# evanwporter/SparseCholesky

Hardware: AMD Instinct MI355X
Metric: numeric-factorization fp64 GFLOP/s (F=sum colcount^2) (higher is better)
Workload: dtype f64

## Files before the change

sparsecholesky_amd/csrc/kernels.hip:

```cpp
#include <hip/hip_runtime.h>

#include <cstdint>
#include <type_traits>

#include "kernels.hpp"

namespace sc {

typedef double double4_t __attribute__((ext_vector_type(4)));

__device__ __forceinline__ void report_fail(int32_t* info, const int32_t* post, int32_t col_internal) {
    atomicMin(info, (post ? post[col_internal] : col_internal) + 1);
}

__device__ __forceinline__ int bnd_at(const int32_t* b, int k, int mbc) {
    const int klo = b[0], khi = b[1];
    return k <= klo ? b[2] : (k >= khi ? mbc : b[2 + k - klo]);
}

__device__ __forceinline__ int lower_bound_i32(const int32_t* a, int n, int v) {
    int lo = 0, hi = n;
    while (lo < hi) {
        int mid = (lo + hi) >> 1;
        if (a[mid] < v)
// ... 11 lines not shown
    const int tid = threadIdx.x;
    const int lane = tid & 63, wid = tid >> 6;
    const int c0 = P.sn_start[s];
    const int w = P.sn_start[s + 1] - c0;
    const int m = P.sn_m[s];
    const int mb = m - w;
    const int j0 = t.y * ASM_COLS;
    const int j1 = min(m, j0 + ASM_COLS);
    double* panel = P.panel_pool + P.panel_off[s];
    double* cbs = P.cb_pool + P.cb_off[s];
    for (int j = j0 + wid; j < j1; j += 4) {
        double* col = (j < w) ? panel + (int64_t)j * m : cbs + (int64_t)(j - w) * mb - w;
#pragma unroll 4
        for (int r = j + lane; r < m; r += 64) col[r] = 0.0;
    }
    __syncthreads();
    for (int j = j0 + wid; j < min(j1, w); j += 4) {
        const int64_t a0 = P.a_ptr[c0 + j], a1 = P.a_ptr[c0 + j + 1];
        for (int64_t q = a0 + lane; q < a1; q += 64) panel[(int64_t)j * m + P.a_pos[q]] = Ax[P.a_src[q]];
    }
    __syncthreads();
    for (int ci = P.child_ptr[s]; ci < P.child_ptr[s + 1]; ++ci) {
        const int c = P.child_list[ci];
        const int mbc = P.sn_m[c] - (P.sn_start[c + 1] - P.sn_start[c]);
        const int32_t* __restrict__ rel = P.relind + P.rel_ptr[c];
        const double* __restrict__ cb = P.cb_pool + P.cb_off[c];
        const int32_t* __restrict__ cbnd = P.col_bnd + P.cbk_ptr[c];
        const int jlo = bnd_at(cbnd, t.y, mbc), jhi = bnd_at(cbnd, t.y + 1, mbc);
        for (int jc = jlo + wid; jc < jhi; jc += 4) {
            const int pj = rel[jc];
            const double* __restrict__ src = cb + (int64_t)jc * mbc;
            double* dst = (pj < w) ? panel + (int64_t)pj * m : cbs + (int64_t)(pj - w) * mb - w;
#pragma unroll 4
            for (int ic = jc + lane; ic < mbc; ic += 64) dst[rel[ic]] += src[ic];
        }
        __syncthreads();
    }
}

constexpr int ASM_CCH = 32;
__global__ __launch_bounds__(256) void assemble_tile_kernel(DevPlan P, const int2* __restrict__ tasks,
                                                             const double* __restrict__ Ax,
                                                             const int2* __restrict__ lim) {
    __shared__ double T[ASM_COLS * ASM_ROWS];
    __shared__ const double* s_src[ASM_CCH];
    __shared__ const int32_t* s_rel[ASM_CCH];
    __shared__ int s_mbc[ASM_CCH], s_ilo[ASM_CCH], s_ihi[ASM_CCH], s_jlo[ASM_CCH];
    __shared__ int8_t s_pj[ASM_CCH][ASM_COLS];
    const int2 t = tasks[blockIdx.x];
    const int s = t.x;
    const int k = t.y >> 16;
    const int jb = t.y & 0xffff;
    const int tid = threadIdx.x;
    const int lane = tid & 63, wid = tid >> 6;
    const int c0 = P.sn_start[s];
    const int w = P.sn_start[s + 1] - c0;
    const int m = P.sn_m[s];
    const int mb = m - w;
    const int j0 = jb * ASM_COLS;
    const int j1 = min(m, j0 + ASM_COLS);
    const int r0 = k * ASM_ROWS, r1 = min(m, r0 + ASM_ROWS);
    const int2 cl = lim ? lim[blockIdx.x] : make_int2(0, m);
    double* panel = P.panel_pool + P.panel_off[s];
    double* cbs = P.cb_pool + P.cb_off[s];
    const int cp0 = P.child_ptr[s], cp1 = P.child_ptr[s + 1];
#pragma unroll
    for (int q = 0; q < ASM_COLS / 4; ++q)
#pragma unroll
        for (int r = lane; r < ASM_ROWS; r += 64) T[(wid + 4 * q) * ASM_ROWS + r] = 0.0;
    for (int j = j0 + wid; j < min(j1, w); j += 4) {
        const int64_t a0 = P.a_ptr[c0 + j], a1 = P.a_ptr[c0 + j + 1];
        for (int64_t q = a0 + lane; q < a1; q += 64) {
            const int p = P.a_pos[q];
            if (p >= r0 && p < r1) T[(j - j0) * ASM_ROWS + (p - r0)] = Ax[P.a_src[q]];
        }
    }
    for (int cb = cp0; cb < cp1; cb += ASM_CCH) {
        const int nc = min(ASM_CCH, cp1 - cb);
        if (cb > cp0) __syncthreads();
        if (tid < nc) {
            const int c = P.child_list[cb + tid];
            const int mbc = P.sn_m[c] - (P.sn_start[c + 1] - P.sn_start[c]);
            const int32_t* rel = P.relind + P.rel_ptr[c];
            const int32_t* bnd = P.rel_bnd + P.rb_ptr[c];
            const int32_t* cbnd = P.col_bnd + P.cbk_ptr[c];
            const int ilo = bnd_at(bnd, k, mbc), ihi = bnd_at(bnd, k + 1, mbc);
            const int jlo = bnd_at(cbnd, jb, mbc), jhi = bnd_at(cbnd, jb + 1, mbc);
            int pj[ASM_COLS];
#pragma unroll
            for (int l = 0; l < ASM_COLS; ++l) {
                const int pc = (jlo + l < jhi && ilo < ihi) ? rel[jlo + l] : -1;
                pj[l] = (pc >= cl.x && pc < cl.y) ? pc - j0 : -1;
            }
#pragma unroll
            for (int l = 0; l < ASM_COLS; ++l) s_pj[tid][l] = (int8_t)pj[l];
            s_src[tid] = P.cb_pool + P.cb_off[c];
            s_rel[tid] = rel;
            s_mbc[tid] = mbc;
            s_ilo[tid] = ilo;
            s_ihi[tid] = ihi;
            s_jlo[tid] = jlo;
        }
        __syncthreads();
        for (int i = 0; i < nc; ++i) {
            const int pjl = lane < ASM_COLS ? (int)s_pj[i][lane] : -1;
            uint64_t mask = __ballot(pjl >= 0 && (pjl & 3) == wid);
            if (!mask) continue;
            const int mbc = s_mbc[i], ilo = s_ilo[i], ihi = s_ihi[i], jlo = s_jlo[i];
            const double* __restrict__ src = s_src[i];
            const int32_t* __restrict__ rel = s_rel[i];
            int jc[4], tc[4];
#pragma unroll
            for (int q = 0; q < 4; ++q) {
                const int b = mask ? __builtin_ctzll(mask) : -1;
                jc[q] = b < 0 ? -1 : jlo + b;
                tc[q] = b < 0 ? 0 : __shfl(pjl, b);
                mask &= mask - 1;
            }
            double v[4][ASM_ROWS / 64];
            int rr[4][ASM_ROWS / 64];
#pragma unroll
            for (int q = 0; q < 4; ++q) {
                const int lo = max(jc[q], ilo) + lane;
#pragma unroll
                for (int ch = 0; ch < ASM_ROWS / 64; ++ch) {
                    const int ic = lo + 64 * ch;
                    const bool ok = jc[q] >= 0 && ic < ihi;
                    rr[q][ch] = ok ? rel[ic] : -1;
                    v[q][ch] = ok ? src[(int64_t)jc[q] * mbc + ic] : 0.0;
                }
            }
#pragma unroll
            for (int q = 0; q < 4; ++q)
#pragma unroll
                for (int ch = 0; ch < ASM_ROWS / 64; ++ch)
                    if (rr[q][ch] >= 0) T[tc[q] * ASM_ROWS + rr[q][ch] - r0] += v[q][ch];
        }
    }
    for (int j = j0 + wid; j < j1; j += 4) {
        if (j < cl.x || j >= cl.y) continue;
        double* col = (j < w) ? panel + (int64_t)j * m : cbs + (int64_t)(j - w) * mb - w;
        const double* Tc = T + (j - j0) * ASM_ROWS - r0;
        for (int r = max(r0, j) + lane; r < r1; r += 64) col[r] = Tc[r];
    }
}

__device__ __forceinline__ __amdgpu_buffer_rsrc_t buf_rsrc(const double* base, uint32_t nbytes = 0xffffffffu) {
    return __builtin_amdgcn_make_buffer_rsrc(const_cast<double*>(base), 0, (int)nbytes, 0x00020000);
}
constexpr int BUF_DEAD = 0x7ffffff0;
__device__ __forceinline__ double buf_ld(__amdgpu_buffer_rsrc_t rs, int voff, int soff) {
    return __builtin_bit_cast(double, __builtin_amdgcn_raw_buffer_load_b64(rs, voff, soff, 0));
}
__device__ __forceinline__ void buf_st(double v, __amdgpu_buffer_rsrc_t rs, int voff, int soff) {
    __builtin_amdgcn_raw_buffer_store_b64(__builtin_bit_cast(decltype(__builtin_amdgcn_raw_buffer_load_b64(rs, 0, 0, 0)), v), rs, voff, soff, 0);
}

__device__ __forceinline__ double readlane_f64(double v, int src) {
    const long long b = __double_as_longlong(v);
    const int lo = __builtin_amdgcn_readlane((int)(b & 0xffffffff), src);
    const int hi = __builtin_amdgcn_readlane((int)(b >> 32), src);
    return __longlong_as_double(((long long)hi << 32) | (unsigned int)lo);
}

template <int J>
__device__ __forceinline__ void trsm_steps(double (&r)[PNB], const double* Lc, const double* invd, int nb) {
    constexpr int LD = PNB + 2;
    if constexpr (J < PNB) {
        if (J < nb) {
            const double rj = r[J] * invd[J];
            r[J] = rj;
#pragma unroll
            for (int q = J + 1; q < PNB; ++q) r[q] = fma(-rj, Lc[J * LD + q], r[q]);
            trsm_steps<J + 1>(r, Lc, invd, nb);
        }
    }
}

__device__ __forceinline__ double rsqrt_f64(double d) {
    double y = __builtin_amdgcn_rsq(d);
    const double h = 0.5 * d;
    y = y * fma(-h * y, y, 1.5);
    y = y * fma(-h * y, y, 1.5);
    return y;
}

__device__ __forceinline__ int pk_col(int m, int j) { return j * m - ((j * (j - 1)) >> 1); }

__device__ __forceinline__ void lds_barrier() { asm volatile("s_waitcnt lgkmcnt(0)\n\ts_barrier" ::: "memory"); }

__device__ __forceinline__ void tile_map(int q, int T, int WT, int& bi, int& bj) {
    const int np = WT * T - WT * (WT - 1) / 2;
    if (q < np) {
        int c = 0, rem = q;
        while (rem >= T - c) {
            rem -= T - c;
            ++c;
        }
        bi = c + rem;
        bj = c;
        return;
    }
    const int r = q - np;
    int b = (int)((sqrtf(8.0f * (float)r + 1.0f) - 1.0f) * 0.5f);
    while (b * (b + 1) / 2 > r) --b;
    while ((b + 1) * (b + 2) / 2 <= r) ++b;
    bi = WT + b;
    bj = WT + r - b * (b + 1) / 2;
}

constexpr int COLB = 132;

template <int KT>
struct SmallRegs {
    double v[KT][16];
    int bi[KT], bj[KT];
};

template <int KT, int NT = 256>
__device__ __forceinline__ void small_tiles(SmallRegs<KT>& R, int m, int w) {
    const int T = (m + 3) >> 2, WT = (w + 3) >> 2, ntile = T * (T + 1) / 2;
#pragma unroll
    for (int k = 0; k < KT; ++k) {
        const int q = threadIdx.x + NT * k;
        int bi = -1, bj = -1;
        if (q < ntile) tile_map(q, T, WT, bi, bj);
        R.bi[k] = bi;
        R.bj[k] = bj;
    }
}

template <int KT>
__device__ __forceinline__ void small_load(SmallRegs<KT>& R, const double* F, int m) {
#pragma unroll
    for (int k = 0; k < KT; ++k)
#pragma unroll
        for (int r = 0; r < 4; ++r)
#pragma unroll
            for (int c = 0; c < 4; ++c) {
                const int i = 4 * R.bi[k] + r, j = 4 * R.bj[k] + c;
                R.v[k][r * 4 + c] = (R.bi[k] >= 0 && i < m && i >= j) ? F[pk_col(m, j) + i - j] : 0.0;
            }
}

template <int KT>
__device__ __forceinline__ void small_steps(SmallRegs<KT>& R, double* colbuf, int w, int32_t* info, const int32_t* post, int c0) {
    for (int J = 0, b = 0; J < w; J += 4, ++b) {
        double* cb = colbuf + (b & 1) * 4 * COLB;
        const int nb = min(4, w - J);
#pragma unroll
        for (int k = 0; k < KT; ++k)
            if (R.bj[k] == b) {
#pragma unroll
                for (int r = 0; r < 4; ++r) {
                    double* row = cb + 4 * (4 * R.bi[k] + r);
                    *reinterpret_cast<double2*>(row) = make_double2(R.v[k][r * 4], R.v[k][r * 4 + 1]);
                    *reinterpret_cast<double2*>(row + 2) = make_double2(R.v[k][r * 4 + 2], R.v[k][r * 4 + 3]);
                }
            }
        lds_barrier();
        double D[4][4];
#pragma unroll
        for (int r = 0; r < 4; ++r) {
            const double2 x01 = *reinterpret_cast<const double2*>(cb + 4 * (J + r));
            const double2 x23 = *reinterpret_cast<const double2*>(cb + 4 * (J + r) + 2);
            D[r][0] = x01.x;
            D[r][1] = x01.y;
            D[r][2] = x23.x;
            D[r][3] = x23.y;
        }
        double Ld[4][4], rc[4];
#pragma unroll
        for (int c = 0; c < 4; ++c) {
            double dd = D[c][c];
#pragma unroll
            for (int t = 0; t < c; ++t) dd = fma(-Ld[c][t], Ld[c][t], dd);
            if (c < nb && threadIdx.x == 0 && !(dd > 0.0)) report_fail(info, post, c0 + J + c);
            rc[c] = c < nb ? rsqrt_f64(dd) : 0.0;
            Ld[c][c] = dd * rc[c];
#pragma unroll
            for (int r = c + 1; r < 4; ++r) {
                double x = D[r][c];
#pragma unroll
                for (int t = 0; t < c; ++t) x = fma(-Ld[r][t], Ld[c][t], x);
                Ld[r][c] = x * rc[c];
            }
        }
        auto solve_row = [&](int row, double (&l)[4]) {
            const double2 x01 = *reinterpret_cast<const double2*>(cb + 4 * row);
            const double2 x23 = *reinterpret_cast<const double2*>(cb + 4 * row + 2);
            const double cr[4] = {x01.x, x01.y, x23.x, x23.y};
#pragma unroll
            for (int k = 0; k < 4; ++k) {
                double x = cr[k];
#pragma unroll
                for (int t = 0; t < k; ++t) x = fma(-l[t], Ld[k][t], x);
                l[k] = x * rc[k];
            }
        };
#pragma unroll
        for (int k = 0; k < KT; ++k) {
            const int bi = R.bi[k], bj = R.bj[k];
            if (bi < 0 || bj < b) continue;
            double lj[4][4];
#pragma unroll
            for (int c = 0; c < 4; ++c) solve_row(4 * bj + c, lj[c]);
// ... 764 lines not shown
                for (int c = 0; c < 4; ++c) {
                    const int i = 4 * R.bi[0] + r, j = 4 * R.bj[0] + c;
                    if (i >= j) Sd[PNB * j - j * (j - 1) / 2 + (i - j)] = (i == j) ? 1.0 / R.v[0][r * 4 + c] : R.v[0][r * 4 + c];
                }
        }
        const int row = r0 + tid;
        const __amdgpu_buffer_rsrc_t rs = buf_rsrc(pan + (int64_t)k0 * m, (uint32_t)m * PNB * 8u);
        const int voff = row < r1 ? row * 8 : BUF_DEAD;
        double r[PNB];
#pragma unroll
        for (int c = 0; c < PNB; ++c) r[c] = buf_ld(rs, voff, c * m * 8);
        __syncthreads();
        trsm64_full(r, S);
#pragma unroll
        for (int c = 0; c < PNB; ++c) buf_st(r[c], rs, voff, c * m * 8);
        return;
    }
    if (SC_POTRF_FAST)
        small_steps1_fast(R, colbuf, PNB, P.info, P.post, c0 + k0);
    else
        small_steps<1>(R, colbuf, PNB, P.info, P.post, c0 + k0);
    if (R.bi[0] >= 0) {
#pragma unroll
        for (int r = 0; r < 4; ++r)
#pragma unroll
            for (int c = 0; c < 4; ++c) {
                const int i = 4 * R.bi[0] + r, j = 4 * R.bj[0] + c;
                if (i >= j) Sd[PNB * j - j * (j - 1) / 2 + (i - j)] = (i == j) ? 1.0 / R.v[0][r * 4 + c] : R.v[0][r * 4 + c];
            }
    }
    const int row = r0 + tid;
    const __amdgpu_buffer_rsrc_t rs = buf_rsrc(pan + (int64_t)k0 * m, (uint32_t)m * PNB * 8u);
    const int voff = row < r1 ? row * 8 : BUF_DEAD;
    double r[PNB];
#pragma unroll
    for (int c = 0; c < PNB; ++c) r[c] = buf_ld(rs, voff, c * m * 8);
    __syncthreads();
    if (tid == 0) {
        const int k1 = k0 + PNB;
        const int nwg = (max(r1, k1 + 1) - k1 + TRSM_ROWS - 1) / TRSM_ROWS;
        const int old = __hip_atomic_fetch_add(arrive + (t.ctr - 1), 1, __ATOMIC_RELAXED, __HIP_MEMORY_SCOPE_AGENT);
        s_last = old == nwg - 1;
        if (old == nwg - 1) __hip_atomic_store(arrive + (t.ctr - 1), 0, __ATOMIC_RELAXED, __HIP_MEMORY_SCOPE_AGENT);
    }
    __syncthreads();
    if (s_last && R.bi[0] >= 0) {
#pragma unroll
        for (int rr = 0; rr < 4; ++rr)
#pragma unroll
            for (int c = 0; c < 4; ++c) {
                const int i = 4 * R.bi[0] + rr, j = 4 * R.bj[0] + c;
                if (i >= j) blk[(int64_t)j * m + i] = R.v[0][rr * 4 + c];
            }
    }
    trsm64_full(r, S);
#pragma unroll
    for (int c = 0; c < PNB; ++c) buf_st(r[c], rs, voff, c * m * 8);
}

#ifndef SC_PROBE_NOGATHER
#define SC_PROBE_NOGATHER 0
#endif
#ifndef SC_PROBE_NOK
#define SC_PROBE_NOK 0
#endif
template <int BT, int WM, int WN, int BK = 16, int GR = 64>
__device__ __forceinline__ void syrk_gather_epilogue(const GemmTask& T, const int64_t* __restrict__ gblk,
                                                     const GSeg* __restrict__ gseg, int row0, int col0,
                                                     double4_t (&acc)[BT / WM / 16][BT / WN / 16], double* smem) {
    constexpr int NW = WM * WN, NT = 64 * NW;
    constexpr int RTM = BT / WM / 16, RTN = BT / WN / 16;
    constexpr int GLD = GR + 1;
    constexpr int GQ = BT == 64 ? (GR == 32 ? 8 : 64 / NW) : SC_GATHER_Q;
    constexpr int SB = BT == 64 ? 4 : 1;
    constexpr int OPS = 2 * 2 * BK * (BT + 16);
    static_assert(BT * GLD <= OPS, "gather chunk fits the operand LDS");
    const int tid = threadIdx.x, lane = tid & 63, wid = tid >> 6;
    const int wr = wid / WN, wc = wid % WN;
    const int w = T.gw;
    const int mb = T.M;
    const int nb = (mb + 63) >> 6;
    const int64_t* __restrict__ blk = gblk + T.gb;
    const GSeg* __restrict__ seg = gseg;
    double* G = smem;
    double* __restrict__ C = T.C;
    const int64_t ldc = T.ldc;
    const __amdgpu_buffer_rsrc_t rc = buf_rsrc(C + (int64_t)col0 * ldc, (uint32_t)(min(BT, T.N - col0) * ldc * 8));
#pragma unroll 1
    for (int h = 0; h < BT / GR; ++h) {
        const int r0 = row0 + h * GR;
        const int rb = r0 >> 6;
        if (h) __syncthreads();
        for (int e = tid; e < BT * GLD; e += NT) G[e] = 0.0;
        __syncthreads();
        const int cb1 = min(min(nb, rb + 1), (col0 + BT) >> 6);
        for (int cbk = col0 >> 6; !SC_PROBE_NOGATHER && r0 < mb && cbk < cb1; ++cbk) {
            const int64_t bi = (int64_t)rb * (rb + 1) / 2 + cbk;
            const int64_t p0 = blk[bi], p1 = blk[bi + 1];
            for (int64_t pb = p0; pb < p1; pb += SB) {
                int prw[SB], pcl[SB];
#pragma unroll
                for (int q = 0; q < SB; ++q) {
                    prw[q] = -1;
                    pcl[q] = -1;
                    if (pb + q < p1) {
                        const GSeg& g = seg[pb + q];
                        const int ic = g.ilo + lane, jl = g.jlo + lane;
                        if (ic < g.ihi) prw[q] = g.rel[ic] - w - r0;
                        if (jl < g.jhi) pcl[q] = g.rel[jl] - w - col0;
                    }
                }
#pragma unroll
                for (int q = 0; q < SB; ++q) {
                    if (pb + q >= p1) break;
                    const GSeg& g = seg[pb + q];
                    const int ic = g.ilo + lane;
                    const int prow = prw[q] < GR ? prw[q] : -1;
                    const int mbc = g.mbc;
                    const double* __restrict__ cb = g.cb;
                    uint64_t mask = __ballot(pcl[q] >= 0 && pcl[q] % NW == wid);
                    while (mask) {
                        int jc[GQ], pc[GQ];
#pragma unroll
                        for (int u = 0; u < GQ; ++u) {
                            const int b = mask ? __builtin_ctzll(mask) : -1;
                            jc[u] = b < 0 ? -1 : g.jlo + b;
                            pc[u] = b < 0 ? 0 : __builtin_amdgcn_readlane(pcl[q], b);
                            mask &= mask - 1;
                        }
                        double v[GQ];
                        bool ok[GQ];
#pragma unroll
                        for (int u = 0; u < GQ; ++u) {
                            ok[u] = jc[u] >= 0 && prow >= 0 && ic >= jc[u];
                            const __amdgpu_buffer_rsrc_t rs = buf_rsrc(cb + (int64_t)max(jc[u], 0) * mbc, (uint32_t)mbc * 8u);
                            v[u] = buf_ld(rs, ok[u] ? ic * 8 : BUF_DEAD, 0);
                        }
#pragma unroll
                        for (int u = 0; u < GQ; ++u)
                            if (ok[u]) G[pc[u] * GLD + prow] += v[u];
                    }
                }
            }
        }
        __syncthreads();
        static_assert(GR % (BT / WM) == 0, "a wave's rows lie in one chunk");
        if ((wr * (BT / WM)) / GR == h) {
#pragma unroll
            for (int a = 0; a < RTM; ++a)
#pragma unroll
                for (int b = 0; b < RTN; ++b)
#pragma unroll
                    for (int r = 0; r < 4; ++r) {
                        const int lr = wr * (BT / WM) + a * 16 + MFMA_F64_ROW(lane, r);
                        const int lc = wc * (BT / WN) + b * 16 + (lane & 15);
                        G[lc * GLD + (lr - h * GR)] -= acc[a][b][r];
                    }
        }
        __syncthreads();
#pragma unroll 4
        for (int e = tid; e < BT * GR; e += NT) {
            const int lr = e % GR, lc = e / GR;
            const int gi = r0 + lr, gj = col0 + lc;
            const bool live = gi < T.M && gi >= gj && gj < T.N;
            buf_st(G[lc * GLD + lr], rc, live ? (int)((gi + (int64_t)(gj - col0) * ldc) * 8) : BUF_DEAD, 0);
        }
    }
}

template <int BT, int WM, int WN, int BK = 16, int GR = 64>
__device__ __forceinline__ void syrk_rmw_epilogue(const GemmTask& T, int row0, int col0,
                                                  double4_t (&acc)[BT / WM / 16][BT / WN / 16], double* smem) {
    constexpr int NW = WM * WN, NT = 64 * NW;
    constexpr int RTM = BT / WM / 16, RTN = BT / WN / 16;
    constexpr int GLD = GR + 1;
    constexpr int OPS = 2 * 2 * BK * (BT + 16);
    static_assert(BT * GLD <= OPS, "chunk fits the operand LDS");
    static_assert(GR % (BT / WM) == 0, "a wave's rows lie in one chunk");
    const int tid = threadIdx.x, lane = tid & 63, wid = tid >> 6;
    const int wr = wid / WN, wc = wid % WN;
    double* G = smem;
    const int64_t ldc = T.ldc;
    const __amdgpu_buffer_rsrc_t rc = buf_rsrc(T.C + (int64_t)col0 * ldc, (uint32_t)(min(BT, T.N - col0) * ldc * 8));
#pragma unroll 1
    for (int h = 0; h < BT / GR; ++h) {
        const int r0 = row0 + h * GR;
        if (h) __syncthreads();
#pragma unroll 4
        for (int e = tid; e < BT * GR; e += NT) {
            const int lr = e % GR, lc = e / GR;
            const int gi = r0 + lr, gj = col0 + lc;
            const bool live = gi < T.M && gi >= gj && gj < T.N;
            G[lc * GLD + lr] = buf_ld(rc, live ? (int)((gi + (int64_t)(gj - col0) * ldc) * 8) : BUF_DEAD, 0);
        }
        __syncthreads();
        if ((wr * (BT / WM)) / GR == h) {
#pragma unroll
            for (int a = 0; a < RTM; ++a)
#pragma unroll
                for (int b = 0; b < RTN; ++b)
#pragma unroll
                    for (int r = 0; r < 4; ++r) {
                        const int lr = wr * (BT / WM) + a * 16 + MFMA_F64_ROW(lane, r);
                        const int lc = wc * (BT / WN) + b * 16 + (lane & 15);
                        G[lc * GLD + (lr - h * GR)] -= acc[a][b][r];
                    }
        }
        __syncthreads();
#pragma unroll 4
        for (int e = tid; e < BT * GR; e += NT) {
            const int lr = e % GR, lc = e / GR;
            const int gi = r0 + lr, gj = col0 + lc;
            const bool live = gi < T.M && gi >= gj && gj < T.N;
            buf_st(G[lc * GLD + lr], rc, live ? (int)((gi + (int64_t)(gj - col0) * ldc) * 8) : BUF_DEAD, 0);
        }
    }
}

template <int BT, int WM, int WN, int BK = 16>
__device__ __forceinline__ void mfma_kloop(const double* __restrict__ A, int64_t lda, int K, int M, int N, int row0,
                                           int col0, double4_t (&acc)[BT / WM / 16][BT / WN / 16], double* smem) {
    static_assert(BK == 16 || BK == 8, "four-deep k sub-steps of the MFMA");
    constexpr int NT = 64 * WM * WN;
    constexpr int LDT = BT + 16;
    constexpr int RTM = BT / WM / 16, RTN = BT / WN / 16;
    double(*As)[BK * LDT] = reinterpret_cast<double(*)[BK * LDT]>(smem);
    double(*Bs)[BK * LDT] = reinterpret_cast<double(*)[BK * LDT]>(smem + 2 * BK * LDT);
    const int tid = threadIdx.x;
    const int lane = tid & 63;
    const int wid = tid >> 6;
    const int wr = wid / WN, wc = wid % WN;
    constexpr int PER = BT * BK / NT;
    double ra[PER], rb[PER];
    auto gload = [&](int k0) {
        const __amdgpu_buffer_rsrc_t rs = buf_rsrc(A + (int64_t)k0 * lda, (uint32_t)(min(BK, K - k0) * lda * 8));
#pragma unroll
        for (int q = 0; q < PER; ++q) {
            const int e = tid + q * NT;
            const int r = e % BT, kk = e / BT;
            const int gr = row0 + r, gc = col0 + r;
            ra[q] = buf_ld(rs, gr < M ? (int)((gr + kk * lda) * 8) : BUF_DEAD, 0);
            rb[q] = buf_ld(rs, gc < N ? (int)((gc + kk * lda) * 8) : BUF_DEAD, 0);
        }
    };
    auto sstore = [&](int buf) {
#pragma unroll
        for (int q = 0; q < PER; ++q) {
            const int e = tid + q * NT;
            const int r = e % BT, kk = e / BT;
            As[buf][kk * LDT + r] = ra[q];
            Bs[buf][kk * LDT + r] = rb[q];
        }
    };

    const int nk = (K + BK - 1) / BK;
    auto stage = [&](int kt, auto last) {
        constexpr bool LAST = decltype(last)::value;
        const int cur = kt & 1;
        if (!LAST) gload((kt + 1) * BK);
        double av[2][RTM], bv[2][RTN];
        auto lread = [&](int kk, int slot) {
            const int krow = kk + (lane >> 4);
#pragma unroll
            for (int a = 0; a < RTM; ++a)
                av[slot][a] = As[cur][krow * LDT + wr * (BT / WM) + a * 16 + (lane & 15)];
#pragma unroll
            for (int b = 0; b < RTN; ++b)
                bv[slot][b] = Bs[cur][krow * LDT + wc * (BT / WN) + b * 16 + (lane & 15)];
        };
        lread(0, 0);
#pragma unroll
        for (int kk = 0; kk < BK; kk += 4) {
            const int slot = (kk / 4) & 1;
            if (kk + 4 < BK) lread(kk + 4, slot ^ 1);
#pragma unroll
            for (int a = 0; a < RTM; ++a)
#pragma unroll
                for (int b = 0; b < RTN; ++b)
                    acc[a][b] = __builtin_amdgcn_mfma_f64_16x16x4f64(av[slot][a], bv[slot][b], acc[a][b], 0, 0, 0);
            if (!LAST && kk == BK - 8) sstore(cur ^ 1);
        }
        __syncthreads();
    };
    gload(0);
    sstore(0);
    __syncthreads();
    for (int kt = 0; kt + 1 < nk; ++kt) stage(kt, std::false_type {});
    if (nk > 0) stage(nk - 1, std::true_type {});
}

template <int BK>
__device__ __forceinline__ void panel_prefactor(const GemmTask& T, int32_t* info, const int32_t* post,
                                                double* smem) {
    static_assert(2 * 2 * BK * (64 + 16) >= 64 * 65 / 2, "the packed diagonal block fits the operand LDS");
    double4_t acc[2][2];
#pragma unroll
    for (int a = 0; a < 2; ++a)
#pragma unroll
        for (int b = 0; b < 2; ++b) acc[a][b] = (double4_t){0.0, 0.0, 0.0, 0.0};
    mfma_kloop<64, 2, 2, BK>(T.A, T.lda, T.K, T.M, T.N, 0, 0, acc, smem);
    const int tid = threadIdx.x, lane = tid & 63, wid = tid >> 6;
    const int wr = wid >> 1, wc = wid & 1;
    const int64_t ldc = T.ldc;
    double* __restrict__ F = smem;
    const __amdgpu_buffer_rsrc_t rc = buf_rsrc(T.C, (uint32_t)(64 * ldc * 8));
    double cv[2][2][4];
#pragma unroll
    for (int a = 0; a < 2; ++a)
#pragma unroll
        for (int b = 0; b < 2; ++b)
#pragma unroll
            for (int r = 0; r < 4; ++r) {
                const int gi = wr * 32 + a * 16 + MFMA_F64_ROW(lane, r), gj = wc * 32 + b * 16 + (lane & 15);
                cv[a][b][r] = buf_ld(rc, gi >= gj ? (int)((gi + (int64_t)gj * ldc) * 8) : BUF_DEAD, 0);
            }
#pragma unroll
    for (int a = 0; a < 2; ++a)
#pragma unroll
        for (int b = 0; b < 2; ++b)
#pragma unroll
            for (int r = 0; r < 4; ++r) {
                const int gi = wr * 32 + a * 16 + MFMA_F64_ROW(lane, r), gj = wc * 32 + b * 16 + (lane & 15);
                if (gi >= gj) F[pk_col(64, gj) + gi - gj] = cv[a][b][r] - acc[a][b][r];
            }
    __syncthreads();
    SmallRegs<1> R;
    small_tiles<1>(R, PNB, PNB);
    small_load<1>(R, F, PNB);
    __syncthreads();
    small_steps1_fast(R, smem, PNB, info, post, T.pf);
    if (R.bi[0] < 0) return;
#pragma unroll
    for (int r = 0; r < 4; ++r)
#pragma unroll
        for (int c = 0; c < 4; ++c) {
            const int i = 4 * R.bi[0] + r, j = 4 * R.bj[0] + c;
            if (i >= j) T.C[(int64_t)j * ldc + i] = R.v[0][r * 4 + c];
        }
}

template <int BT, int WM, int WN, int TAG, int EPI, int LEAN = 0, int PF = 0>
__device__ __forceinline__ void syrk_tile_body(const GemmTask* __restrict__ tasks, const int2* __restrict__ tiles,
                                               int bidx, const int64_t* __restrict__ gblk,
                                               const GSeg* __restrict__ gseg, int32_t* info = nullptr,
                                               const int32_t* post = nullptr) {
    constexpr int BK = LEAN ? 8 : 16;
    constexpr int LDT = BT + 16;
    constexpr int RTM = BT / WM / 16, RTN = BT / WN / 16;
    __shared__ __attribute__((aligned(16))) double smem[2 * 2 * BK * LDT];

    const int2 tl = tiles[bidx];
    const GemmTask T = tasks[tl.x];
    if constexpr (PF) {
        static_assert(BT == 64 && WM == 2 && WN == 2 && TAG == 0, "pre-factor on 64 x 64 panel-update tiles");
        if (tl.y < 0) {
            panel_prefactor<BK>(T, info, post, smem);
            return;
        }
    }
    const int ti = tl.y >> 16, tj = tl.y & 0xffff;
    const int row0 = ti * BT, col0 = tj * BT;

    const int wid = threadIdx.x >> 6;
    if (wid >= WM * WN / 2) __builtin_amdgcn_s_setprio(1);

    double4_t acc[RTM][RTN];
#pragma unroll
    for (int a = 0; a < RTM; ++a)
#pragma unroll
        for (int b = 0; b < RTN; ++b) acc[a][b] = (double4_t){0.0, 0.0, 0.0, 0.0};
    if (!(SC_PROBE_NOK && TAG == 1 && T.gs >= 0)) mfma_kloop<BT, WM, WN, BK>(T.A, T.lda, T.K, T.M, T.N, row0, col0, acc, smem);

    if constexpr (TAG == 1) {
        if (T.gs >= 0) {
            syrk_gather_epilogue<BT, WM, WN, BK, LEAN ? 32 : 64>(T, gblk, gseg, row0, col0, acc, smem);
            return;
        }
    }
    syrk_rmw_epilogue<BT, WM, WN, BK, LEAN ? 32 : 64>(T, row0, col0, acc, smem);
}

template <int BT, int WM, int WN, int TAG, int EPI, int LEAN = 0, int PF = 0>
__global__ __launch_bounds__(64 * WM * WN, LEAN ? (TAG ? 5 : 6) : 1) void syrk_mfma_kernel(const GemmTask* __restrict__ tasks,
                                                                  const int2* __restrict__ tiles,
                                                                  const int64_t* __restrict__ gblk,
                                                                  const GSeg* __restrict__ gseg, int32_t* info,
                                                                  const int32_t* post) {
    syrk_tile_body<BT, WM, WN, TAG, EPI, LEAN, PF>(tasks, tiles, blockIdx.x, gblk, gseg, info, post);
}

static int small_kt(int maxm) {
    const int T = (maxm + 3) / 4;
    return (T * (T + 1) / 2 + 255) / 256;
}

hipError_t launch_front_small(const DevPlan& P, const int32_t* nodes, int count, int maxm, bool seq,
                              const double* Ax, hipStream_t st) {
    if (count <= 0) return hipSuccess;
    const size_t lds = (size_t)maxm * (maxm + 1) / 2 * sizeof(double);
    const int kt = small_kt(maxm);
    const dim3 grid(seq ? 1 : count);
    const int sq = seq ? count : 0;
    if (kt <= 1)
        hipLaunchKernelGGL(front_small_kernel<1>, grid, dim3(256), lds, st, P, nodes, Ax, sq);
    else if (kt == 2)
        hipLaunchKernelGGL(front_small_kernel<2>, grid, dim3(256), lds, st, P, nodes, Ax, sq);
    else
        hipLaunchKernelGGL(front_small_kernel<3>, grid, dim3(256), lds, st, P, nodes, Ax, sq);
    return hipGetLastError();
}

hipError_t launch_front_chain(const DevPlan& P, const ChainPlan& C, int first, int count, int maxm,
                              const double* Ax, hipStream_t st) {
    if (count <= 0) return hipSuccess;
    if (count > CHAIN_MAXF || maxm > 128) return hipErrorInvalidValue;
    const int fsz = maxm * (maxm + 1) / 2;
    const size_t lds = (size_t)fsz * sizeof(double);
    hipLaunchKernelGGL(chain_init_kernel, dim3(count), dim3(256), lds, st, P, C, first, Ax);
    hipLaunchKernelGGL(front_chain_kernel, dim3(1), dim3(CHAIN_NT), (SC_CHAIN_DB ? 2 : 1) * lds, st, P, C, first, count,
                       fsz);
    return hipGetLastError();
}

hipError_t launch_assemble_large(const DevPlan& P, const int2* tasks, int count, const double* Ax,
                                 hipStream_t st, bool tiled, const int2* lim) {
    if (count <= 0) return hipSuccess;
    if (tiled)
        hipLaunchKernelGGL(assemble_tile_kernel, dim3(count), dim3(256), 0, st, P, tasks, Ax, lim);
    else
        hipLaunchKernelGGL(assemble_cols_kernel, dim3(count), dim3(256), 0, st, P, tasks, Ax);
    return hipGetLastError();
}

hipError_t launch_potrf_diag(const DevPlan& P, const int2* tasks, int count, hipStream_t st) {
    if (count <= 0) return hipSuccess;
    hipLaunchKernelGGL(potrf_tiles_kernel, dim3(count), dim3(256), 0, st, P, tasks);
    return hipGetLastError();
}

hipError_t launch_trsm_panel(const DevPlan& P, const TrsmTask* tasks, int count, hipStream_t st, bool partial,
                             int32_t* arrive, int pre) {
    if (count <= 0) return hipSuccess;
    if (partial)
        hipLaunchKernelGGL(trsm_partial_kernel, dim3(count), dim3(TRSM_ROWS), 0, st, P, tasks);
    else if (pre == 2)
        hipLaunchKernelGGL(trsm_panel_g_kernel<2>, dim3(count), dim3(TRSM_ROWS), 0, st, P, tasks, arrive);
    else
        hipLaunchKernelGGL(trsm_panel_g_kernel<0>, dim3(count), dim3(TRSM_ROWS), 0, st, P, tasks, arrive);
    return hipGetLastError();
}

template <int TAG, int EPI>
static void launch_syrk_t(const GemmTask* tasks, const int2* tiles, int n, int bt, hipStream_t st, GatherTab gt,
                          bool lean) {
    if (bt == 64 && lean)
        hipLaunchKernelGGL((syrk_mfma_kernel<64, 2, 2, TAG, EPI, 1>), dim3(n), dim3(256), 0, st, tasks, tiles, gt.blk,
                           gt.seg, gt.info, gt.post);
    else if (bt == 128)
        hipLaunchKernelGGL((syrk_mfma_kernel<128, 2, 4, TAG, EPI>), dim3(n), dim3(512), 0, st, tasks, tiles, gt.blk,
                           gt.seg, gt.info, gt.post);
    else
        hipLaunchKernelGGL((syrk_mfma_kernel<64, 2, 2, TAG, EPI>), dim3(n), dim3(256), 0, st, tasks, tiles, gt.blk,
                           gt.seg, gt.info, gt.post);
}

hipError_t launch_syrk(const GemmTask* tasks, const int2* tiles, int total_tiles, int bt, int tag, hipStream_t st,
                       int epi, GatherTab gt, bool lean, bool pf) {
    if (total_tiles <= 0) return hipSuccess;
    if (pf) {
        if (bt != 64 || tag) return hipErrorInvalidValue;
        hipLaunchKernelGGL((syrk_mfma_kernel<64, 2, 2, 0, 1, 0, 1>), dim3(total_tiles), dim3(256), 0, st, tasks, tiles,
                           gt.blk, gt.seg, gt.info, gt.post);
        return hipGetLastError();
    }
    if (tag)
        epi ? launch_syrk_t<1, 1>(tasks, tiles, total_tiles, bt, st, gt, lean)
            : launch_syrk_t<1, 0>(tasks, tiles, total_tiles, bt, st, gt, lean);
    else
        epi ? launch_syrk_t<0, 1>(tasks, tiles, total_tiles, bt, st, gt, lean)
            : launch_syrk_t<0, 0>(tasks, tiles, total_tiles, bt, st, gt, lean);
    return hipGetLastError();
}

__global__ void fill_random_kernel(double* p, int64_t n) {
    for (int64_t i = blockIdx.x * (int64_t)blockDim.x + threadIdx.x; i < n; i += (int64_t)gridDim.x * blockDim.x) {
        uint64_t x = (uint64_t)i * 0x9E3779B97F4A7C15ull;
        x ^= x >> 31;
        x *= 0xBF58476D1CE4E5B9ull;
        x ^= x >> 29;
        p[i] = (double)(x >> 11) * (2.0 / 9007199254740992.0) - 1.0;
    }
}

hipError_t launch_fill_random(double* p, int64_t n, hipStream_t st) {
    hipLaunchKernelGGL(fill_random_kernel, dim3(1024), dim3(256), 0, st, p, n);
    return hipGetLastError();
}

__global__ void stamp_kernel(uint64_t* slot) { *slot = __builtin_amdgcn_s_memrealtime(); }

__global__ void status_publish_kernel(int32_t* info, int32_t* host) {
    const int32_t v = __hip_atomic_load(info, __ATOMIC_RELAXED, __HIP_MEMORY_SCOPE_AGENT);
    __hip_atomic_store(info, 0x7f7f7f7f, __ATOMIC_RELAXED, __HIP_MEMORY_SCOPE_AGENT);
    __hip_atomic_store(host, v, __ATOMIC_RELEASE, __HIP_MEMORY_SCOPE_SYSTEM);
}

hipError_t launch_status_publish(int32_t* info, int32_t* host, hipStream_t st) {
    hipLaunchKernelGGL(status_publish_kernel, dim3(1), dim3(1), 0, st, info, host);
    return hipGetLastError();
}

__global__ void hwid_kernel(uint32_t* out, int spin) {
    if (threadIdx.x == 0) {
        out[2 * blockIdx.x] = __builtin_amdgcn_s_getreg((31 << 11) | 4);
        out[2 * blockIdx.x + 1] = __builtin_amdgcn_s_getreg((15 << 11) | 20);
    }
    const uint64_t t0 = __builtin_amdgcn_s_memrealtime();
    while (__builtin_amdgcn_s_memrealtime() - t0 < (uint64_t)spin) __builtin_amdgcn_s_sleep(8);
}

hipError_t launch_hwid(uint32_t* out, int nwg, int threads, int spin, hipStream_t st) {
    hipLaunchKernelGGL(hwid_kernel, dim3(nwg), dim3(threads), 0, st, out, spin);
    return hipGetLastError();
}

hipError_t launch_stamp(uint64_t* slot, hipStream_t st) {
    hipLaunchKernelGGL(stamp_kernel, dim3(1), dim3(1), 0, st, slot);
    return hipGetLastError();
}

__global__ __launch_bounds__(256) void copy2d_kernel(const Copy2D* __restrict__ descs, const int2* __restrict__ tiles,
                                                     int unpack) {
    const int2 t = tiles[blockIdx.x];
    const Copy2D d = descs[t.x];
    const int lane = threadIdx.x & 63, wid = threadIdx.x >> 6;
    const int j0 = t.y & 0xffff, r0 = (t.y >> 16) * COPY_ROWS;
// ... 2245 lines not shown
```

sparsecholesky_amd/csrc/kernels.hpp:

```cpp
#pragma once

#include <hip/hip_runtime.h>

#include <cstdint>
#include <vector>

namespace sc {

constexpr int PNB = 64;
constexpr int TRSM_ROWS = 256;
constexpr int ASM_COLS = 16;
constexpr int ASM_ROWS = 256;
constexpr int ASM_TILE_MIN_M = 512;
constexpr int SYRK_BT_SMALL = 64;
constexpr int SYRK_BT_LARGE = 128;

#define MFMA_F64_ROW(lane, r) (((lane) >> 4) + 4 * (r))

#ifndef SC_GATHER_Q
#define SC_GATHER_Q 4
#endif

struct DevPlan {
    const int32_t* sn_start;
    const int32_t* sn_m;
    const int64_t* panel_off;
    const int64_t* cb_off;
    const int32_t* child_ptr;
    const int32_t* child_list;
    const int64_t* rel_ptr;
    const int32_t* relind;
    const int64_t* rb_ptr;
    const int32_t* rel_bnd;
    const int64_t* cbk_ptr;
    const int32_t* col_bnd;
    const int64_t* tb_ptr;
    const int32_t* tile_bnd;
    const int64_t* a_ptr;
    const int32_t* a_pos;
    const int64_t* a_src;
    double* panel_pool;
    double* cb_pool;
    int32_t* info;
    const int32_t* post;
};

struct GSeg {
    const double* cb;
    const int32_t* rel;
    int32_t mbc, ilo, ihi, jlo, jhi, pad;
};

struct GatherTab {
    const int64_t* blk = nullptr;
    const GSeg* seg = nullptr;
    int32_t* info = nullptr;
    const int32_t* post = nullptr;
};

struct GemmTask {
    double* C;
    const double* A;
    int64_t ldc;
    int64_t lda;
    int32_t M, N, K;
    int32_t gs = -1, gv = 0;
    int64_t gb = -1;
    int32_t gw = 0;
    int32_t pf = -1;
};
struct Copy2D {
    double* a;
    double* b;
    int64_t lda;
    int32_t rows, cols;
};

constexpr int COPY_COLS = 16;
constexpr int COPY_ROWS = 2048;
constexpr int COPY_MAX_COLS = 32768;
static_assert(COPY_MAX_COLS + COPY_COLS <= 65536, "column offsets fit the tile's 16 low bits");
hipError_t launch_copy2d(const Copy2D* descs, const int2* tiles, int count, bool unpack, hipStream_t st);

struct SolvePlan {
    const int32_t* sn_start;
    const int32_t* sn_m;
    const int64_t* panel_off;
    const int64_t* rows_ptr;
    const int32_t* rows;
    const double* panel_pool;
    double* c;
    double* y;
    double* u;
    const int64_t* u_off;
    const int32_t* child_ptr;
    const int32_t* child_list;
    const int64_t* rel_ptr;
    const int32_t* relind;
    double* part;
};
constexpr int SOLVE_ROWS = 256;
constexpr int SOLVE_NB = 128;
hipError_t launch_solve_inv(const SolvePlan& P, const int2* tasks, int count, const int2* tasks2, int count2,
                            hipStream_t st);
hipError_t launch_solve_fwd(const SolvePlan& P, const int4* tasks, int count, hipStream_t st);
hipError_t launch_solve_fwd_gather(const SolvePlan& P, const int32_t* fronts, int count, hipStream_t st);
hipError_t launch_solve_gemv(const SolvePlan& P, const int4* tasks, int count, hipStream_t st);
hipError_t launch_solve_diag(const SolvePlan& P, const int4* tasks, int count, hipStream_t st);
hipError_t launch_permute(double* dst, const double* src, const int32_t* perm, int64_t n, bool scatter,
                          hipStream_t st);

constexpr int SOLVE_RHS = 16;
hipError_t launch_solve_fwd_multi(const SolvePlan& P, const int4* tasks, int count, hipStream_t st);
hipError_t launch_solve_fwd_gather_multi(const SolvePlan& P, const int32_t* fronts, int count, hipStream_t st);
hipError_t launch_solve_gemv_multi(const SolvePlan& P, const int4* tasks, int count, hipStream_t st);
hipError_t launch_solve_diag_multi(const SolvePlan& P, const int4* tasks, int count, hipStream_t st);
hipError_t launch_permute_multi(double* c, double* io, const int32_t* perm, int64_t n, bool scatter,
                                hipStream_t st);

hipError_t launch_mul_l_multi(const SolvePlan& P, const int4* tasks, int count, hipStream_t st);
hipError_t launch_mul_lt_gemv_multi(const SolvePlan& P, const int4* tasks, int count, hipStream_t st);
hipError_t launch_mul_lt_diag_multi(const SolvePlan& P, const int4* tasks, int count, hipStream_t st);
constexpr int LOGDET_NT = 256;
hipError_t launch_logdet(const SolvePlan& P, int ns, int64_t n, double* part, double* out, hipStream_t st);

struct SelBlk {
    int32_t s, k0;
    int64_t woff;
};
struct SelPlan {
    const int32_t* sn_start;
    const int32_t* sn_m;
    const int64_t* panel_off;
    const int64_t* cb_off;
    const int64_t* rel_ptr;
    const int32_t* relind;
    const double* lpanel;
    double* zpanel;
    double* zii;
    double* wbuf;
    double* part;
    const SelBlk* blk;
};
constexpr int SEL_NW = 4;
constexpr int SEL_BM = 16 * SEL_NW;
constexpr int SEL_KT = 64;
constexpr int SEL_BK = 16;
constexpr int SEL_KC = 256, SEL_KSPLIT = 512;
inline int selinv_kchunks(int64_t K) { return K <= SEL_KSPLIT ? 1 : (int)((K + SEL_KC - 1) / SEL_KC); }
hipError_t launch_selinv_w(const SelPlan& P, const int2* tiles, int count, hipStream_t st);
hipError_t launch_selinv_zrk(const SelPlan& P, const int2* tiles, int count, hipStream_t st);
hipError_t launch_selinv_zkk(const SelPlan& P, const int4* tasks, int count, const int4* red, int nred,
                             hipStream_t st);
hipError_t launch_selinv_push(const SelPlan& P, const int4* tasks, int count, hipStream_t st);
hipError_t launch_selinv_diag(const SelPlan& P, int ns, int64_t n, const int32_t* post, double* diag, hipStream_t st);

constexpr int UPD_W = 16;
constexpr int UPD_K = PNB + UPD_W;
constexpr int UPD_ROWS = 64;
constexpr int32_t UPD_ARMED = 0x7f7f7f7f;
struct UpdPlan {
    const int32_t* sn_start;
    const int32_t* sn_m;
    const int64_t* panel_off;
    const int64_t* rows_ptr;
    const int32_t* rows;
    double* panel_pool;
    double* wd;
    double* tbuf;
    int32_t* info;
// ... 176 lines not shown
```

Baseline: 58000.

## Interleave MFMA tile pairs for 128-bit LDS reads in SYRK k-loop

Remaps which rows and columns each MFMA sub-tile covers so that two adjacent 16-wide tiles interleave. Each lane can then fetch its A and B operands for a tile pair with one 16-byte LDS read instead of two 8-byte reads. The LDS padding is removed (LDT = BT), and every epilogue index is rewritten through new row and column macros to match the interleaved accumulator layout. The occupancy hint for the LEAN TAG=1 variant also rises from 5 to 6, which risks register pressure, and the unpadded stride may bring back LDS bank conflicts.

Result: no change. 58280, median of 6 (+0.5%).

```diff
diff --git a/sparsecholesky_amd/csrc/kernels.hip b/sparsecholesky_amd/csrc/kernels.hip
--- a/sparsecholesky_amd/csrc/kernels.hip
+++ b/sparsecholesky_amd/csrc/kernels.hip
@@ -187,6 +187,7 @@
 __device__ __forceinline__ double buf_ld(__amdgpu_buffer_rsrc_t rs, int voff, int soff) {
     return __builtin_bit_cast(double, __builtin_amdgcn_raw_buffer_load_b64(rs, voff, soff, 0));
 }
+typedef double double2_t __attribute__((ext_vector_type(2)));
 __device__ __forceinline__ void buf_st(double v, __amdgpu_buffer_rsrc_t rs, int voff, int soff) {
     __builtin_amdgcn_raw_buffer_store_b64(__builtin_bit_cast(decltype(__builtin_amdgcn_raw_buffer_load_b64(rs, 0, 0, 0)), v), rs, voff, soff, 0);
 }
@@ -1257,8 +1258,8 @@
                 for (int b = 0; b < RTN; ++b)
 #pragma unroll
                     for (int r = 0; r < 4; ++r) {
-                        const int lr = wr * (BT / WM) + a * 16 + MFMA_F64_ROW(lane, r);
-                        const int lc = wc * (BT / WN) + b * 16 + (lane & 15);
+                        const int lr = wr * (BT / WM) + SYRK_ACC_ROW(a, lane, r);
+                        const int lc = wc * (BT / WN) + SYRK_ACC_COL(b, lane);
                         G[lc * GLD + (lr - h * GR)] -= acc[a][b][r];
                     }
         }
@@ -1306,8 +1307,8 @@
                 for (int b = 0; b < RTN; ++b)
 #pragma unroll
                     for (int r = 0; r < 4; ++r) {
-                        const int lr = wr * (BT / WM) + a * 16 + MFMA_F64_ROW(lane, r);
-                        const int lc = wc * (BT / WN) + b * 16 + (lane & 15);
+                        const int lr = wr * (BT / WM) + SYRK_ACC_ROW(a, lane, r);
+                        const int lc = wc * (BT / WN) + SYRK_ACC_COL(b, lane);
                         G[lc * GLD + (lr - h * GR)] -= acc[a][b][r];
                     }
         }
@@ -1327,8 +1328,9 @@
                                            int col0, double4_t (&acc)[BT / WM / 16][BT / WN / 16], double* smem) {
     static_assert(BK == 16 || BK == 8, "four-deep k sub-steps of the MFMA");
     constexpr int NT = 64 * WM * WN;
-    constexpr int LDT = BT + 16;
+    constexpr int LDT = BT;
     constexpr int RTM = BT / WM / 16, RTN = BT / WN / 16;
+    static_assert(RTM % 2 == 0 && RTN % 2 == 0, "MFMA tiles pair up into 32-row groups");
     double(*As)[BK * LDT] = reinterpret_cast<double(*)[BK * LDT]>(smem);
     double(*Bs)[BK * LDT] = reinterpret_cast<double(*)[BK * LDT]>(smem + 2 * BK * LDT);
     const int tid = threadIdx.x;
@@ -1367,11 +1369,19 @@
         auto lread = [&](int kk, int slot) {
             const int krow = kk + (lane >> 4);
 #pragma unroll
-            for (int a = 0; a < RTM; ++a)
-                av[slot][a] = As[cur][krow * LDT + wr * (BT / WM) + a * 16 + (lane & 15)];
-#pragma unroll
-            for (int b = 0; b < RTN; ++b)
-                bv[slot][b] = Bs[cur][krow * LDT + wc * (BT / WN) + b * 16 + (lane & 15)];
+            for (int g = 0; g < RTM / 2; ++g) {
+                const double2_t v = *reinterpret_cast<const double2_t*>(
+                    &As[cur][krow * LDT + wr * (BT / WM) + g * 32 + 2 * (lane & 15)]);
+                av[slot][2 * g] = v.x;
+                av[slot][2 * g + 1] = v.y;
+            }
+#pragma unroll
+            for (int g = 0; g < RTN / 2; ++g) {
+                const double2_t v = *reinterpret_cast<const double2_t*>(
+                    &Bs[cur][krow * LDT + wc * (BT / WN) + g * 32 + 2 * (lane & 15)]);
+                bv[slot][2 * g] = v.x;
+                bv[slot][2 * g + 1] = v.y;
+            }
         };
         lread(0, 0);
 #pragma unroll
@@ -1416,7 +1426,7 @@
         for (int b = 0; b < 2; ++b)
 #pragma unroll
             for (int r = 0; r < 4; ++r) {
-                const int gi = wr * 32 + a * 16 + MFMA_F64_ROW(lane, r), gj = wc * 32 + b * 16 + (lane & 15);
+                const int gi = wr * 32 + SYRK_ACC_ROW(a, lane, r), gj = wc * 32 + SYRK_ACC_COL(b, lane);
                 cv[a][b][r] = buf_ld(rc, gi >= gj ? (int)((gi + (int64_t)gj * ldc) * 8) : BUF_DEAD, 0);
             }
 #pragma unroll
@@ -1425,7 +1435,7 @@
         for (int b = 0; b < 2; ++b)
 #pragma unroll
             for (int r = 0; r < 4; ++r) {
-                const int gi = wr * 32 + a * 16 + MFMA_F64_ROW(lane, r), gj = wc * 32 + b * 16 + (lane & 15);
+                const int gi = wr * 32 + SYRK_ACC_ROW(a, lane, r), gj = wc * 32 + SYRK_ACC_COL(b, lane);
                 if (gi >= gj) F[pk_col(64, gj) + gi - gj] = cv[a][b][r] - acc[a][b][r];
             }
     __syncthreads();
@@ -1486,7 +1496,7 @@
 }
 
 template <int BT, int WM, int WN, int TAG, int EPI, int LEAN = 0, int PF = 0>
-__global__ __launch_bounds__(64 * WM * WN, LEAN ? (TAG ? 5 : 6) : 1) void syrk_mfma_kernel(const GemmTask* __restrict__ tasks,
+__global__ __launch_bounds__(64 * WM * WN, LEAN ? 6 : 1) void syrk_mfma_kernel(const GemmTask* __restrict__ tasks,
                                                                   const int2* __restrict__ tiles,
                                                                   const int64_t* __restrict__ gblk,
                                                                   const GSeg* __restrict__ gseg, int32_t* info,
diff --git a/sparsecholesky_amd/csrc/kernels.hpp b/sparsecholesky_amd/csrc/kernels.hpp
--- a/sparsecholesky_amd/csrc/kernels.hpp
+++ b/sparsecholesky_amd/csrc/kernels.hpp
@@ -16,6 +16,8 @@
 constexpr int SYRK_BT_LARGE = 128;
 
 #define MFMA_F64_ROW(lane, r) (((lane) >> 4) + 4 * (r))
+#define SYRK_ACC_ROW(a, lane, r) (((a) >> 1) * 32 + 2 * MFMA_F64_ROW(lane, r) + ((a) & 1))
+#define SYRK_ACC_COL(b, lane) (((b) >> 1) * 32 + 2 * ((lane) & 15) + ((b) & 1))
 
 #ifndef SC_GATHER_Q
 #define SC_GATHER_Q 4
```
